# EPFL-VILAB/MultiMAE

Hardware: NVIDIA H100
Metric: MultiMAE-B pretrain samples/sec @ bs=128/GPU (higher is better)
Workload: dtype bf16

## Files before the change

multimae_b200/csrc/gemm_wgmma.cu:

```cuda
#include <algorithm>
#include <cstdlib>

#include "common.cuh"
#include "../../include/multimae_b200.h"

namespace mmae {

void count_launch();
bool gemm_profile_begin(cudaStream_t st, double flops, int M, int N, int K, int flags);
void gemm_profile_end(cudaStream_t st);

namespace {

constexpr int BM = 128;
constexpr int BK = 64;
constexpr int WG_K = 16;
constexpr int GEMM_THREADS = 384;

struct GemmParams {
  int M, N, K;
  int num_kb;
  int kb_per_split;
  int tiles_n;
  int tiles_m;
  int splits;
  int tma_store;
  mmae_gemm_epilogue ep;
};

template <int BN>
struct GemmCfg {
  static constexpr int STAGES = BN == 256 ? 4 : (BN == 192 ? 4 : (BN == 128 ? 6 : 8));
  static constexpr int A_BYTES = BM * BK * 2;
  static constexpr int B_BYTES = BN * BK * 2;
  static constexpr int STAGE_BYTES = A_BYTES + B_BYTES;
  static constexpr int EPI_BOX_BYTES = 64 * 32 * 4;
  static constexpr int EPI_OFFSET = STAGES * STAGE_BYTES;
  static constexpr int BAR_OFFSET = EPI_OFFSET + 2 * 2 * EPI_BOX_BYTES;
  static constexpr int TOTAL = BAR_OFFSET + 256 + 1024;
  static_assert(TOTAL <= 232448, "GEMM exceeds the 227 KB shared-memory limit");
};

struct WorkItem {
  int m0, n0, split, kb_begin, nkb;
};

template <int BN, int CL>
__device__ __forceinline__ WorkItem decode_item(int item, const GemmParams& p, int rank) {
  WorkItem w;
  const int rest = item / p.tiles_n;
  w.n0 = (item - rest * p.tiles_n) * BN;
  w.split = rest / p.tiles_m;
  w.m0 = ((rest - w.split * p.tiles_m) * CL + rank) * BM;
  w.kb_begin = w.split * p.kb_per_split;
  w.nkb = min(p.kb_per_split, p.num_kb - w.kb_begin);
  return w;
}

__device__ __forceinline__ void red_add_v2(float* addr, float a, float b) {
  asm volatile("red.global.add.v2.f32 [%0], {%1, %2};" ::"l"(addr), "f"(a), "f"(b) : "memory");
}

__device__ __forceinline__ void epilogue_pair(float v0, float v1, int row, int n, const GemmParams& p, bool first_split,
                                              bool atomic_out) {
  const mmae_gemm_epilogue& ep = p.ep;
  v0 *= ep.alpha;
  v1 *= ep.alpha;
  if (ep.bias && first_split) {
    const float2 b = __ldg(reinterpret_cast<const float2*>(ep.bias + n));
    v0 += b.x;
    v1 += b.y;
  }
  if (ep.preact_bf16)
    *reinterpret_cast<uint32_t*>(reinterpret_cast<bf16*>(ep.preact_bf16) + int64_t(row) * ep.ld_preact + n) = pack_bf16x2(v0, v1);
  if (ep.act == 1) {
    v0 = gelu_erf(v0);
    v1 = gelu_erf(v1);
  }
  if (ep.dgelu_z) {
    const uint32_t z = __ldg(reinterpret_cast<const unsigned int*>(reinterpret_cast<const bf16*>(ep.dgelu_z) +
                                                                   int64_t(row) * ep.ld_dgelu_z + n));
    const float2 zf = unpack_bf16x2(z);
    v0 *= dgelu_erf(zf.x);
    v1 *= dgelu_erf(zf.y);
  }
  if (ep.residual && first_split) {
    const float2 r = __ldg(reinterpret_cast<const float2*>(ep.residual + int64_t(row) * ep.ld_residual + n));
    v0 += r.x;
    v1 += r.y;
  }
  if (ep.out_f32) {
    float* dst = ep.out_f32 + int64_t(row) * ep.ld_out_f32 + n;
    if (atomic_out) red_add_v2(dst, v0, v1);
    else *reinterpret_cast<float2*>(dst) = make_float2(v0, v1);
  }
  if (ep.out_bf16)
    *reinterpret_cast<uint32_t*>(reinterpret_cast<bf16*>(ep.out_bf16) + int64_t(row) * ep.ld_out_bf16 + n) = pack_bf16x2(v0, v1);
}

template <typename T>
__device__ __forceinline__ void stage_pair(uint8_t* box, int r, int c, float v0, float v1) {
  T* b = reinterpret_cast<T*>(box);
  if constexpr (sizeof(T) == 4) *reinterpret_cast<float2*>(b + r * 32 + c) = make_float2(v0, v1);
  else *reinterpret_cast<uint32_t*>(b + r * 32 + c) = pack_bf16x2(v0, v1);
}

template <int BN, int CL, bool A_MN, bool B_MN>
__global__ void __launch_bounds__(GEMM_THREADS, 1)
    gemm_bf16_kernel(const __grid_constant__ CUtensorMap tmA, const __grid_constant__ CUtensorMap tmB,
                     const __grid_constant__ CUtensorMap tmC, const GemmParams p) {
  pdl_launch_dependents();
  using C = GemmCfg<BN>;
  constexpr int STAGES = C::STAGES;
  constexpr int BH = BN / CL;
  static_assert(!B_MN || BH % 64 == 0, "MN-major B is loaded in 64-column chunks");

  extern __shared__ uint8_t smem_raw[];
  const uint32_t raw_addr = smem_u32(smem_raw);
  uint8_t* smem = smem_raw + ((1024u - (raw_addr & 1023u)) & 1023u);
  uint64_t* full_bar = reinterpret_cast<uint64_t*>(smem + C::BAR_OFFSET);
  uint64_t* empty_bar = full_bar + STAGES;

  const int wg = threadIdx.x >> 7;
  const int rank = CL > 1 ? int(cluster_ctarank()) : 0;
  const int num_items = p.tiles_n * p.tiles_m * p.splits;
  const int first_item = blockIdx.x / CL;
  const int item_stride = gridDim.x / CL;

  if (threadIdx.x == 0) {
    tma_prefetch_desc(&tmA);
    tma_prefetch_desc(&tmB);
    if (p.tma_store) tma_prefetch_desc(&tmC);
#pragma unroll
    for (int s = 0; s < STAGES; ++s) {
      mbar_init(&full_bar[s], 1);
      mbar_init(&empty_bar[s], 2 * CL);
    }
    fence_barrier_init();
  }
  __syncthreads();
  if constexpr (CL > 1) cluster_sync_all();
  pdl_wait();

  if (wg == 0) {
    setmaxnreg_dec<40>();
    if (threadIdx.x == 0) {
      uint32_t it = 0;
      for (int item = first_item; item < num_items; item += item_stride) {
        const WorkItem w = decode_item<BN, CL>(item, p, rank);
        for (int kb = 0; kb < w.nkb; ++kb, ++it) {
          const int s = it % STAGES;
          const uint32_t ph = (it / STAGES) & 1;
          mbar_wait(&empty_bar[s], ph ^ 1u);
          mbar_expect_tx(&full_bar[s], C::STAGE_BYTES);
          uint8_t* sA = smem + s * C::STAGE_BYTES;
          uint8_t* sB = sA + C::A_BYTES;
          const int k0 = (w.kb_begin + kb) * BK;
          if constexpr (!A_MN) {
            tma_load_2d(sA, &tmA, &full_bar[s], k0, w.m0);
          } else {
#pragma unroll
            for (int c = 0; c < BM / 64; ++c) tma_load_2d(sA + c * (64 * BK * 2), &tmA, &full_bar[s], w.m0 + c * 64, k0);
          }
          if constexpr (CL == 1) {
            if constexpr (!B_MN) {
              tma_load_2d(sB, &tmB, &full_bar[s], k0, w.n0);
            } else {
#pragma unroll
              for (int c = 0; c < BN / 64; ++c) tma_load_2d(sB + c * (64 * BK * 2), &tmB, &full_bar[s], w.n0 + c * 64, k0);
            }
          } else {
            if constexpr (!B_MN) {
              tma_load_2d_multicast(sB + rank * BH * 128, &tmB, &full_bar[s], k0, w.n0 + rank * BH, 0x3);
            } else {
#pragma unroll
              for (int c = 0; c < BH / 64; ++c)
                tma_load_2d_multicast(sB + (rank * (BH / 64) + c) * (64 * BK * 2), &tmB, &full_bar[s],
                                      w.n0 + rank * BH + c * 64, k0, 0x3);
            }
          }
        }
      }
    }
  } else {
    setmaxnreg_inc<232>();
    const int cw = wg - 1;
    const int t = threadIdx.x & 127;
    const int rl = (t >> 5) * 16 + ((t & 31) >> 2);
    uint8_t* epi = smem + C::EPI_OFFSET + cw * (2 * C::EPI_BOX_BYTES);
    const bool atomic_out = p.ep.accumulate != 0 || p.splits > 1;
    uint32_t it = 0;
    uint32_t boxes = 0;
    auto release = [&](int s) {
      if (t == 0) {
        if constexpr (CL == 1) mbar_arrive(&empty_bar[s]);
        else
          for (int r = 0; r < CL; ++r) mbar_arrive_cluster(mapa_u32(smem_u32(&empty_bar[s]), uint32_t(r)));
      }
    };
    float acc[BN / 2];

    for (int item = first_item; item < num_items; item += item_stride) {
      const WorkItem w = decode_item<BN, CL>(item, p, rank);
      for (int kb = 0; kb < w.nkb; ++kb, ++it) {
        const int s = it % STAGES;
        const uint32_t ph = (it / STAGES) & 1;
        mbar_wait(&full_bar[s], ph);
        const uint32_t a_addr = smem_u32(smem + s * C::STAGE_BYTES) + cw * (64 * BK * 2);
        const uint32_t b_addr = smem_u32(smem + s * C::STAGE_BYTES) + C::A_BYTES;
#pragma unroll
        for (int i = 0; i < BN / 2; ++i) reg_fence(acc[i]);
        wgmma_fence();
#pragma unroll
        for (int j = 0; j < BK / WG_K; ++j) {
          const uint32_t sd = (kb | j) != 0 ? 1u : 0u;
          const uint64_t da = A_MN ? gmma_desc_sw128(a_addr + j * (WG_K * 128), 64 * BK * 2, 1024)
                                   : gmma_desc_sw128(a_addr + j * (WG_K * 2), 16, 1024);
          const uint64_t db = B_MN ? gmma_desc_sw128(b_addr + j * (WG_K * 128), 64 * BK * 2, 1024)
                                   : gmma_desc_sw128(b_addr + j * (WG_K * 2), 16, 1024);
          if constexpr (BN == 256) wgmma_m64n256k16<A_MN ? 1 : 0, B_MN ? 1 : 0>(acc, da, db, sd);
          else if constexpr (BN == 192) wgmma_m64n192k16<A_MN ? 1 : 0, B_MN ? 1 : 0>(acc, da, db, sd);
          else if constexpr (BN == 128) wgmma_m64n128k16<A_MN ? 1 : 0, B_MN ? 1 : 0>(acc, da, db, sd);
          else wgmma_m64n64k16<A_MN ? 1 : 0, B_MN ? 1 : 0>(acc, da, db, sd);
        }
        wgmma_commit();
#pragma unroll
        for (int i = 0; i < BN / 2; ++i) reg_fence(acc[i]);
        wgmma_wait<1>();
        if (kb > 0) release((it - 1) % STAGES);
      }
      wgmma_wait<0>();
#pragma unroll
      for (int i = 0; i < BN / 2; ++i) reg_fence(acc[i]);
      release((it - 1) % STAGES);

      const int row_a = w.m0 + cw * 64 + rl;
      const int row_b = row_a + 8;
      const bool first_split = w.split == 0;
      if (p.tma_store) {
        const float* bias = first_split ? p.ep.bias : nullptr;
        const bool bf16_out = p.tma_store == 1;
#pragma unroll
        for (int b = 0; b < BN / 32; ++b) {
          if (w.n0 + b * 32 >= p.N) break;
          uint8_t* box = bf16_out ? epi + (boxes & 3) * (C::EPI_BOX_BYTES / 2) : epi + (boxes & 1) * C::EPI_BOX_BYTES;
          if (t == 0) {
            if (bf16_out) bulk_wait_read<3>();
            else bulk_wait_read<1>();
          }
          asm volatile("bar.sync %0, 128;" ::"r"(2 + cw) : "memory");
#pragma unroll
          for (int jj = 0; jj < 4; ++jj) {
            const int j = 4 * b + jj;
            const int c = jj * 8 + 2 * (t & 3);
            float v[4] = {acc[4 * j] * p.ep.alpha, acc[4 * j + 1] * p.ep.alpha, acc[4 * j + 2] * p.ep.alpha,
                          acc[4 * j + 3] * p.ep.alpha};
            if (bias && w.n0 + b * 32 + c < p.N) {
              const float2 bb = __ldg(reinterpret_cast<const float2*>(bias + w.n0 + b * 32 + c));
              v[0] += bb.x; v[1] += bb.y; v[2] += bb.x; v[3] += bb.y;
            }
            if (p.ep.act == 1) {
#pragma unroll
              for (int i = 0; i < 4; ++i) v[i] = gelu_erf(v[i]);
            }
            if (bf16_out) {
              stage_pair<bf16>(box, rl, c, v[0], v[1]);
              stage_pair<bf16>(box, rl + 8, c, v[2], v[3]);
            } else {
              stage_pair<float>(box, rl, c, v[0], v[1]);
              stage_pair<float>(box, rl + 8, c, v[2], v[3]);
            }
          }
          fence_proxy_async_smem();
          asm volatile("bar.sync %0, 128;" ::"r"(2 + cw) : "memory");
          if (t == 0) {
            if (p.tma_store == 3) tma_reduce_add_2d(&tmC, box, w.n0 + b * 32, w.m0 + cw * 64);
            else tma_store_2d(&tmC, box, w.n0 + b * 32, w.m0 + cw * 64);
            bulk_commit_group();
          }
          ++boxes;
        }
      } else {
#pragma unroll
        for (int j = 0; j < BN / 8; ++j) {
          if (w.n0 + j * 8 >= p.N) break;
          const int n = w.n0 + j * 8 + 2 * (t & 3);
          if (row_a < p.M) epilogue_pair(acc[4 * j], acc[4 * j + 1], row_a, n, p, first_split, atomic_out);
          if (row_b < p.M) epilogue_pair(acc[4 * j + 2], acc[4 * j + 3], row_b, n, p, first_split, atomic_out);
        }
      }
    }
    if (t == 0 && p.tma_store) bulk_wait_all();
  }
  if constexpr (CL > 1) cluster_sync_all();
}

template <int BN, int CL, bool A_MN, bool B_MN>
int launch_gemm(const CUtensorMap& tmA, const CUtensorMap& tmB, const CUtensorMap& tmC, const GemmParams& p,
                cudaStream_t stream) {
  using C = GemmCfg<BN>;
  auto kern = gemm_bf16_kernel<BN, CL, A_MN, B_MN>;
  cudaLaunchConfig_t cfg;
  memset(&cfg, 0, sizeof(cfg));
  cfg.blockDim = dim3(GEMM_THREADS);
  cfg.dynamicSmemBytes = C::TOTAL;
  cfg.stream = stream;
  cudaLaunchAttribute attr[2];
  attr[0].id = cudaLaunchAttributeClusterDimension;
  attr[0].val.clusterDim.x = CL;
  attr[0].val.clusterDim.y = 1;
  attr[0].val.clusterDim.z = 1;
  attr[1].id = cudaLaunchAttributeProgrammaticStreamSerialization;
  attr[1].val.programmaticStreamSerializationAllowed = 1;
  cfg.attrs = attr;
  cfg.numAttrs = 1;
  static int resident = 0;
  if (resident == 0) {
    MMAE_CUDA_OK(cudaFuncSetAttribute(kern, cudaFuncAttributeMaxDynamicSharedMemorySize, C::TOTAL));
    if constexpr (CL > 1) {
      cfg.gridDim = dim3(CL);
      MMAE_CUDA_OK(cudaOccupancyMaxActiveClusters(&resident, kern, &cfg));
    } else {
      int dev = 0, sms = 0;
      MMAE_CUDA_OK(cudaGetDevice(&dev));
      MMAE_CUDA_OK(cudaDeviceGetAttribute(&sms, cudaDevAttrMultiProcessorCount, dev));
      resident = sms;
    }
    MMAE_CHECK(resident > 0, MMAE_ERR_CUDA, "mmae_gemm_bf16: the GEMM kernel does not fit on an SM");
  }
  const int items = p.tiles_n * p.tiles_m * p.splits;
  const int slots = std::min(resident, std::max(1, sm_count() / CL));
  cfg.gridDim = dim3(std::min(items, slots) * CL);
  const bool prof = gemm_profile_begin(stream, 2.0 * p.M * p.N * p.K, p.M, p.N, p.K,
                                       (A_MN ? 1 : 0) | (B_MN ? 2 : 0) | (p.splits << 8));
  if constexpr (CL == 1) {
    cfg.attrs = attr + 1;
    cfg.numAttrs = pdl_enabled() ? 1 : 0;
  } else {
    cfg.numAttrs = pdl_enabled() ? 2 : 1;
  }
  MMAE_CUDA_OK(cudaLaunchKernelEx(&cfg, kern, tmA, tmB, tmC, p));
  if (prof) gemm_profile_end(stream);
  count_launch();
  MMAE_LAUNCH_OK();
  return MMAE_OK;
}

}
}

using namespace mmae;

static int g_gemm_variant = []() {
  const char* e = getenv("MMAE_GEMM_VARIANT");
  const int v = e ? atoi(e) : -1;
  return v >= -1 && v <= 6 ? v : -1;
}();
static int g_gemm_tma_store = []() {
  const char* e = getenv("MMAE_GEMM_TMA_STORE");
  return e ? (atoi(e) != 0) : 1;
}();

extern "C" int mmae_gemm_set_variant(int variant) {
  MMAE_CHECK(variant >= -1 && variant <= 6, MMAE_ERR_ARG, "mmae_gemm_set_variant: %d (-1 .. 6)", variant);
  g_gemm_variant = variant;
  return MMAE_OK;
}

extern "C" int mmae_gemm_set_tma_store(int enable) {
  g_gemm_tma_store = enable != 0;
  return MMAE_OK;
}

static int variant_bn(int v) { return v == 0 ? 64 : (v == 1 || v == 6) ? 128 : (v == 3 || v == 5) ? 192 : 256; }

constexpr int KB_PER_ITEM_FIXED = 4;
constexpr int MIN_KB_PER_SPLIT = 16;

extern "C" int mmae_gemm_bf16(const void* A, int64_t lda, int a_mn_major, const void* B, int64_t ldb,
                              int b_mn_major, int M, int N, int K, int split_k, const mmae_gemm_epilogue* ep,
                              void* stream) {
  MMAE_CHECK(A && B && ep, MMAE_ERR_ARG, "mmae_gemm_bf16: null operand");
  MMAE_CHECK(M > 0 && N > 0 && K > 0, MMAE_ERR_ARG, "mmae_gemm_bf16: bad shape M=%d N=%d K=%d", M, N, K);
  MMAE_CHECK(N % 8 == 0, MMAE_ERR_ARG, "mmae_gemm_bf16: N=%d must be a multiple of 8", N);
  MMAE_CHECK(lda % 8 == 0 && ldb % 8 == 0, MMAE_ERR_ARG, "mmae_gemm_bf16: lda/ldb must be multiples of 8");
  MMAE_CHECK((reinterpret_cast<uintptr_t>(A) & 15) == 0 && (reinterpret_cast<uintptr_t>(B) & 15) == 0,
             MMAE_ERR_ARG, "mmae_gemm_bf16: operands must be 16-byte aligned");
  MMAE_CHECK(ep->out_f32 || ep->out_bf16, MMAE_ERR_ARG, "mmae_gemm_bf16: no output");
  const int num_kb = ceil_div(K, BK);
  const int sms = sm_count();
  const int tm = ceil_div(M, BM);
  if (split_k <= 0 && !(ep->out_f32 && !ep->out_bf16 && !ep->preact_bf16 && !ep->dgelu_z && ep->act == 0)) split_k = 1;

  int variant = g_gemm_variant;
  {
    const int cand_var[2] = {1, 2};
    const int nvar = variant >= 0 ? 1 : 2;
    long best_cost = -1;
    int best_split = 1, best_var = variant >= 0 ? variant : 1;
    for (int i = 0; i < nvar; ++i) {
      const int v = variant >= 0 ? variant : cand_var[i];
      const int bn = variant_bn(v), cl = v >= 4 ? 2 : 1;
      if (variant < 0 && bn > 128 && N < bn) continue;
      const long tiles = long(ceil_div(tm, cl)) * ceil_div(N, bn);
      const int slots = std::max(1, sms / cl);
      const int s_lo = split_k > 0 ? split_k : 1;
      const int s_hi = split_k > 0 ? split_k : std::max(1, num_kb / MIN_KB_PER_SPLIT);
      for (int s = s_lo; s <= s_hi; ++s) {
        const int kbps = ceil_div(num_kb, std::min(s, num_kb));
        const long rounds = (tiles * ceil_div(num_kb, kbps) + slots - 1) / slots;
        const long cost = rounds * (bn + 40) * cl * (kbps + KB_PER_ITEM_FIXED);
        if (best_cost < 0 || cost < best_cost) {
          best_cost = cost;
          best_split = s;
          best_var = v;
        }
      }
    }
    split_k = best_split;
    variant = best_var;
  }
  if (split_k > num_kb) split_k = num_kb;
  const int kb_per_split = ceil_div(num_kb, split_k);
  split_k = ceil_div(num_kb, kb_per_split);
  if (split_k > 1 || ep->accumulate) {
    MMAE_CHECK(ep->out_f32 && !ep->out_bf16 && !ep->preact_bf16 && !ep->dgelu_z && ep->act == 0, MMAE_ERR_ARG,
               "mmae_gemm_bf16: split-K / accumulate supports only a linear fp32 epilogue");
  }
#define MMAE_LD_OK(ptr, ld) (!(ptr) || ((ld) % 8 == 0 && (reinterpret_cast<uintptr_t>(ptr) & 15) == 0))
  MMAE_CHECK(MMAE_LD_OK(ep->residual, ep->ld_residual) && MMAE_LD_OK(ep->dgelu_z, ep->ld_dgelu_z) &&
                 MMAE_LD_OK(ep->preact_bf16, ep->ld_preact) && MMAE_LD_OK(ep->out_f32, ep->ld_out_f32) &&
                 MMAE_LD_OK(ep->out_bf16, ep->ld_out_bf16) &&
                 (!ep->bias || (reinterpret_cast<uintptr_t>(ep->bias) & 15) == 0),
             MMAE_ERR_ARG, "mmae_gemm_bf16: epilogue tensors need 16-byte alignment and ld %% 8 == 0");
#undef MMAE_LD_OK

  if (variant == 5 && b_mn_major) variant = 4;
  const int BNsel = variant_bn(variant);
  const int CLsel = variant >= 4 ? 2 : 1;

  CUtensorMap tmA, tmB;
  int rc;
  if (!a_mn_major) {
    rc = make_tmap_2d_bf16(&tmA, A, (uint64_t)M, (uint64_t)K, (uint64_t)lda, BK, BM);
  } else {
    MMAE_CHECK(M % 8 == 0, MMAE_ERR_ARG, "mmae_gemm_bf16: MN-major A needs M %% 8 == 0");
    rc = make_tmap_2d_bf16(&tmA, A, (uint64_t)K, (uint64_t)M, (uint64_t)lda, 64, BK);
  }
  if (rc) return rc;
  if (!b_mn_major) {
    rc = make_tmap_2d_bf16(&tmB, B, (uint64_t)N, (uint64_t)K, (uint64_t)ldb, BK, BNsel / CLsel);
  } else {
    rc = make_tmap_2d_bf16(&tmB, B, (uint64_t)K, (uint64_t)N, (uint64_t)ldb, 64, BK);
  }
  if (rc) return rc;

  GemmParams p;
  p.M = M; p.N = N; p.K = K;
  p.num_kb = num_kb;
  p.kb_per_split = kb_per_split;
  p.tiles_n = ceil_div(N, BNsel);
  p.tiles_m = ceil_div(tm, CLsel);
  p.splits = split_k;
  p.ep = *ep;
  p.tma_store = 0;
  CUtensorMap tmC = tmA;
  if (g_gemm_tma_store && !ep->preact_bf16 && !ep->dgelu_z && !ep->residual) {
    if (ep->out_bf16 && !ep->out_f32 && split_k == 1 && !ep->accumulate) {
      p.tma_store = 1;
      rc = make_tmap_2d_store(&tmC, ep->out_bf16, 2, (uint64_t)M, (uint64_t)N, (uint64_t)ep->ld_out_bf16);
      if (rc) return rc;
    } else if (ep->out_f32 && !ep->out_bf16 && ep->act == 0) {
      p.tma_store = (split_k > 1 || ep->accumulate) ? 3 : 2;
      rc = make_tmap_2d_store(&tmC, ep->out_f32, 4, (uint64_t)M, (uint64_t)N, (uint64_t)ep->ld_out_f32);
      if (rc) return rc;
    }
  }
  cudaStream_t st = reinterpret_cast<cudaStream_t>(stream);
#define MMAE_DISPATCH(BN_, CL_)                                                                      \
  do {                                                                                               \
    if (!a_mn_major && !b_mn_major) return launch_gemm<BN_, CL_, false, false>(tmA, tmB, tmC, p, st); \
    if (!a_mn_major && b_mn_major) return launch_gemm<BN_, CL_, false, true>(tmA, tmB, tmC, p, st);   \
    if (a_mn_major && !b_mn_major) return launch_gemm<BN_, CL_, true, false>(tmA, tmB, tmC, p, st);   \
    return launch_gemm<BN_, CL_, true, true>(tmA, tmB, tmC, p, st);                                  \
  } while (0)
  if (variant == 4) MMAE_DISPATCH(256, 2);
  if (variant == 6) MMAE_DISPATCH(128, 2);
  if (variant == 5) {
    if (!a_mn_major) return launch_gemm<192, 2, false, false>(tmA, tmB, tmC, p, st);
    return launch_gemm<192, 2, true, false>(tmA, tmB, tmC, p, st);
  }
  if (variant == 0) MMAE_DISPATCH(64, 1);
  if (variant == 3) MMAE_DISPATCH(192, 1);
  if (variant == 2) MMAE_DISPATCH(256, 1);
  MMAE_DISPATCH(128, 1);
#undef MMAE_DISPATCH
}
```

multimae_b200/csrc/runtime.cu:

```cuda
#include <atomic>
#include <cstdarg>
#include <cstdio>
#include <cstring>
#include <vector>

#include "common.cuh"
#include "../../include/multimae_b200.h"

namespace mmae {

static thread_local char g_err[512] = "";
static std::atomic<int64_t> g_launches{0};

void set_last_error(const char* fmt, ...) {
  va_list ap;
  va_start(ap, fmt);
  vsnprintf(g_err, sizeof(g_err), fmt, ap);
  va_end(ap);
}

void count_launch() { g_launches.fetch_add(1, std::memory_order_relaxed); }

struct GemmProfile {
  bool on = false;
  std::vector<cudaEvent_t> begin, end;
  std::vector<double> flops;
  std::vector<long long> shape;
  size_t used = 0;
};
static GemmProfile g_prof;
static const size_t kProfCap = 8192;

bool gemm_profile_begin(cudaStream_t st, double flops, int M, int N, int K, int flags) {
  if (!g_prof.on || g_prof.used >= kProfCap) return false;
  if (g_prof.begin.size() <= g_prof.used) {
    cudaEvent_t a, b;
    if (cudaEventCreate(&a) != cudaSuccess || cudaEventCreate(&b) != cudaSuccess) return false;
    g_prof.begin.push_back(a);
    g_prof.end.push_back(b);
    g_prof.flops.push_back(0.0);
    for (int i = 0; i < 4; ++i) g_prof.shape.push_back(0);
  }
  g_prof.flops[g_prof.used] = flops;
  g_prof.shape[4 * g_prof.used + 0] = M;
  g_prof.shape[4 * g_prof.used + 1] = N;
  g_prof.shape[4 * g_prof.used + 2] = K;
  g_prof.shape[4 * g_prof.used + 3] = flags;
  cudaEventRecord(g_prof.begin[g_prof.used], st);
  return true;
}
void gemm_profile_end(cudaStream_t st) {
  cudaEventRecord(g_prof.end[g_prof.used], st);
  g_prof.used++;
}

static int g_sm_budget = []() {
  const char* e = getenv("MMAE_SM_BUDGET");
  return e ? atoi(e) : 0;
}();
int sm_count() {
  static int cached = 0;
  if (cached == 0) {
    int dev = 0;
    cudaGetDevice(&dev);
    cudaDeviceGetAttribute(&cached, cudaDevAttrMultiProcessorCount, dev);
    if (cached <= 0) cached = 132;
  }
  return g_sm_budget > 0 && g_sm_budget < cached ? g_sm_budget : cached;
}

typedef CUresult (*encode_tiled_fn)(CUtensorMap*, CUtensorMapDataType, cuuint32_t, void*, const cuuint64_t*,
                                    const cuuint64_t*, const cuuint32_t*, const cuuint32_t*,
                                    CUtensorMapInterleave, CUtensorMapSwizzle, CUtensorMapL2promotion,
                                    CUtensorMapFloatOOBfill);

static encode_tiled_fn get_encode_fn() {
  static encode_tiled_fn fn = nullptr;
  if (!fn) {
    void* p = nullptr;
    cudaDriverEntryPointQueryResult q;
    cudaError_t e = cudaGetDriverEntryPoint("cuTensorMapEncodeTiled", &p, cudaEnableDefault, &q);
    if (e != cudaSuccess || q != cudaDriverEntryPointSuccess || !p) {
      set_last_error("cuTensorMapEncodeTiled entry point unavailable (%s)", cudaGetErrorString(e));
      return nullptr;
    }
    fn = reinterpret_cast<encode_tiled_fn>(p);
  }
  return fn;
}

int make_tmap_2d_bf16(CUtensorMap* out, const void* base, uint64_t rows, uint64_t cols, uint64_t ld,
                      uint32_t box_cols, uint32_t box_rows) {
  encode_tiled_fn fn = get_encode_fn();
  if (!fn) return MMAE_ERR_CUDA;
  cuuint64_t dims[2] = {cols, rows};
  cuuint64_t strides[1] = {ld * 2};
  cuuint32_t box[2] = {box_cols, box_rows};
  cuuint32_t estr[2] = {1, 1};
  CUresult r = fn(out, CU_TENSOR_MAP_DATA_TYPE_BFLOAT16, 2, const_cast<void*>(base), dims, strides, box, estr,
                  CU_TENSOR_MAP_INTERLEAVE_NONE, CU_TENSOR_MAP_SWIZZLE_128B, CU_TENSOR_MAP_L2_PROMOTION_L2_256B,
                  CU_TENSOR_MAP_FLOAT_OOB_FILL_NONE);
  if (r != CUDA_SUCCESS) {
    set_last_error("cuTensorMapEncodeTiled(2d) failed: %d (rows=%llu cols=%llu ld=%llu box=%ux%u base=%p)", (int)r,
                   (unsigned long long)rows, (unsigned long long)cols, (unsigned long long)ld, box_cols, box_rows,
                   base);
    return MMAE_ERR_CUDA;
  }
  return MMAE_OK;
}

int make_tmap_2d_store(CUtensorMap* out, const void* base, int elem_bytes, uint64_t rows, uint64_t cols, uint64_t ld) {
  encode_tiled_fn fn = get_encode_fn();
  if (!fn) return MMAE_ERR_CUDA;
  cuuint64_t dims[2] = {cols, rows};
  cuuint64_t strides[1] = {ld * (uint64_t)elem_bytes};
  cuuint32_t box[2] = {32, 64};
  cuuint32_t estr[2] = {1, 1};
  CUresult r = fn(out, elem_bytes == 2 ? CU_TENSOR_MAP_DATA_TYPE_BFLOAT16 : CU_TENSOR_MAP_DATA_TYPE_FLOAT32, 2,
                  const_cast<void*>(base), dims, strides, box, estr,
                  CU_TENSOR_MAP_INTERLEAVE_NONE, CU_TENSOR_MAP_SWIZZLE_NONE, CU_TENSOR_MAP_L2_PROMOTION_NONE,
                  CU_TENSOR_MAP_FLOAT_OOB_FILL_NONE);
  if (r != CUDA_SUCCESS) {
    set_last_error("cuTensorMapEncodeTiled(store) failed: %d (rows=%llu cols=%llu ld=%llu base=%p)", (int)r,
                   (unsigned long long)rows, (unsigned long long)cols, (unsigned long long)ld, base);
    return MMAE_ERR_CUDA;
  }
  return MMAE_OK;
}

int make_tmap_3d_bf16(CUtensorMap* out, const void* base, uint64_t d0, uint64_t d1, uint64_t d2, uint64_t s1,
                      uint64_t s2, uint32_t b0, uint32_t b1, uint32_t b2) {
  encode_tiled_fn fn = get_encode_fn();
  if (!fn) return MMAE_ERR_CUDA;
  cuuint64_t dims[3] = {d0, d1, d2};
  cuuint64_t strides[2] = {s1 * 2, s2 * 2};
  cuuint32_t box[3] = {b0, b1, b2};
  cuuint32_t estr[3] = {1, 1, 1};
  CUresult r = fn(out, CU_TENSOR_MAP_DATA_TYPE_BFLOAT16, 3, const_cast<void*>(base), dims, strides, box, estr,
                  CU_TENSOR_MAP_INTERLEAVE_NONE, CU_TENSOR_MAP_SWIZZLE_128B, CU_TENSOR_MAP_L2_PROMOTION_L2_256B,
                  CU_TENSOR_MAP_FLOAT_OOB_FILL_NONE);
  if (r != CUDA_SUCCESS) {
    set_last_error("cuTensorMapEncodeTiled(3d) failed: %d", (int)r);
    return MMAE_ERR_CUDA;
  }
  return MMAE_OK;
}

int make_tmap_3d_bf16_store(CUtensorMap* out, const void* base, uint64_t d0, uint64_t d1, uint64_t d2, uint64_t s1,
                            uint64_t s2, uint32_t b0, uint32_t b1, uint32_t b2) {
  encode_tiled_fn fn = get_encode_fn();
  if (!fn) return MMAE_ERR_CUDA;
  cuuint64_t dims[3] = {d0, d1, d2};
  cuuint64_t strides[2] = {s1 * 2, s2 * 2};
  cuuint32_t box[3] = {b0, b1, b2};
  cuuint32_t estr[3] = {1, 1, 1};
  const CUtensorMapSwizzle sw = b0 * 2 == 128 ? CU_TENSOR_MAP_SWIZZLE_128B : (b0 * 2 == 64 ? CU_TENSOR_MAP_SWIZZLE_64B : CU_TENSOR_MAP_SWIZZLE_NONE);
  CUresult r = fn(out, CU_TENSOR_MAP_DATA_TYPE_BFLOAT16, 3, const_cast<void*>(base), dims, strides, box, estr,
                  CU_TENSOR_MAP_INTERLEAVE_NONE, sw, CU_TENSOR_MAP_L2_PROMOTION_NONE, CU_TENSOR_MAP_FLOAT_OOB_FILL_NONE);
  if (r != CUDA_SUCCESS) {
    set_last_error("cuTensorMapEncodeTiled(3d store) failed: %d", (int)r);
    return MMAE_ERR_CUDA;
  }
  return MMAE_OK;
}

}

namespace mmae {
namespace {
struct MirrorEntry {
  const float* f32;
  bf16* b16;
  int64_t n;
};
constexpr int MAX_MIRRORS = 8;
MirrorEntry g_mirror[MAX_MIRRORS];
int g_num_mirrors = 0;
}

const bf16* mirror_lookup(const float* w) {
  for (int i = 0; i < g_num_mirrors; ++i) {
    const MirrorEntry& e = g_mirror[i];
    if (w >= e.f32 && w < e.f32 + e.n) {
      const int64_t off = w - e.f32;
      if (off % 8 != 0) return nullptr;
      return e.b16 + off;
    }
  }
  return nullptr;
}
}

extern "C" int mmae_weight_mirror_register(const float* params_f32, void* mirror_bf16, int64_t n) {
  using namespace mmae;
  MMAE_CHECK(params_f32 != nullptr, MMAE_ERR_ARG, "mmae_weight_mirror_register: null parameter buffer");
  int at = -1;
  for (int i = 0; i < g_num_mirrors; ++i)
    if (g_mirror[i].f32 == params_f32) at = i;
  if (mirror_bf16 == nullptr || n <= 0) {
    if (at >= 0) g_mirror[at] = g_mirror[--g_num_mirrors];
    return MMAE_OK;
  }
  MMAE_CHECK((reinterpret_cast<uintptr_t>(params_f32) & 31) == 0 && (reinterpret_cast<uintptr_t>(mirror_bf16) & 15) == 0,
             MMAE_ERR_ARG, "mmae_weight_mirror_register: buffers must be 32-byte (fp32) / 16-byte (bf16) aligned");
  if (at < 0) {
    MMAE_CHECK(g_num_mirrors < MAX_MIRRORS, MMAE_ERR_UNSUPPORTED, "mmae_weight_mirror_register: too many mirrors");
    at = g_num_mirrors++;
  }
  g_mirror[at] = {params_f32, reinterpret_cast<bf16*>(mirror_bf16), n};
  return MMAE_OK;
}

namespace mmae {
static int g_pdl = []() {
  const char* e = getenv("MMAE_PDL");
  return e ? atoi(e) : 0;
}();
bool pdl_enabled() { return g_pdl != 0; }
}
extern "C" int mmae_set_sm_budget(int sms) {
  mmae::g_sm_budget = sms;
  return MMAE_OK;
}
extern "C" int mmae_set_pdl(int enable) {
  mmae::g_pdl = enable != 0;
  return MMAE_OK;
}

extern "C" int mmae_abi_version(void) { return MMAE_ABI_VERSION; }
extern "C" const char* mmae_last_error(void) { return mmae::g_err; }
extern "C" int64_t mmae_launch_count(void) { return mmae::g_launches.load(std::memory_order_relaxed); }

extern "C" int mmae_profile_gemm(int enable) {
  mmae::g_prof.on = enable != 0;
  if (enable) mmae::g_prof.used = 0;
  return MMAE_OK;
}
extern "C" int mmae_profile_gemm_read(double* flops, double* ms, int64_t* launches) {
  double f = 0.0, t = 0.0;
  for (size_t i = 0; i < mmae::g_prof.used; ++i) {
    if (cudaEventSynchronize(mmae::g_prof.end[i]) != cudaSuccess) return MMAE_ERR_CUDA;
    float e = 0.f;
    if (cudaEventElapsedTime(&e, mmae::g_prof.begin[i], mmae::g_prof.end[i]) != cudaSuccess) return MMAE_ERR_CUDA;
    t += e;
    f += mmae::g_prof.flops[i];
  }
  if (flops) *flops = f;
  if (ms) *ms = t;
  if (launches) *launches = (int64_t)mmae::g_prof.used;
  return MMAE_OK;
}

extern "C" int64_t mmae_profile_gemm_dump(char* buf, int64_t cap) {
  int64_t off = 0;
  for (size_t i = 0; i < mmae::g_prof.used; ++i) {
    if (cudaEventSynchronize(mmae::g_prof.end[i]) != cudaSuccess) return -1;
    float e = 0.f;
    cudaEventElapsedTime(&e, mmae::g_prof.begin[i], mmae::g_prof.end[i]);
    const int n = snprintf(buf + off, (size_t)(cap - off), "%lld %lld %lld %lld %.6f\n", mmae::g_prof.shape[4 * i],
                           mmae::g_prof.shape[4 * i + 1], mmae::g_prof.shape[4 * i + 2], mmae::g_prof.shape[4 * i + 3], e);
    if (n <= 0 || off + n >= cap) break;
    off += n;
  }
  return off;
}
```

Baseline: 3886.

## Swizzle TMA-store epilogue boxes and lend a pipeline stage for BN=256 staging

```diff
diff --git a/multimae_b200/csrc/gemm_wgmma.cu b/multimae_b200/csrc/gemm_wgmma.cu
--- a/multimae_b200/csrc/gemm_wgmma.cu
+++ b/multimae_b200/csrc/gemm_wgmma.cu
@@ -31,12 +31,13 @@
 template <int BN>
 struct GemmCfg {
   static constexpr int STAGES = BN == 256 ? 4 : (BN == 192 ? 4 : (BN == 128 ? 6 : 8));
+  static constexpr int EPI_BOXES = 2;
   static constexpr int A_BYTES = BM * BK * 2;
   static constexpr int B_BYTES = BN * BK * 2;
   static constexpr int STAGE_BYTES = A_BYTES + B_BYTES;
-  static constexpr int EPI_BOX_BYTES = 64 * 32 * 4;
+  static constexpr int EPI_BOX_BYTES = 64 * 128;
   static constexpr int EPI_OFFSET = STAGES * STAGE_BYTES;
-  static constexpr int BAR_OFFSET = EPI_OFFSET + 2 * 2 * EPI_BOX_BYTES;
+  static constexpr int BAR_OFFSET = EPI_OFFSET + 2 * EPI_BOXES * EPI_BOX_BYTES;
   static constexpr int TOTAL = BAR_OFFSET + 256 + 1024;
   static_assert(TOTAL <= 232448, "GEMM exceeds the 227 KB shared-memory limit");
 };
@@ -100,9 +101,60 @@
 
 template <typename T>
 __device__ __forceinline__ void stage_pair(uint8_t* box, int r, int c, float v0, float v1) {
-  T* b = reinterpret_cast<T*>(box);
-  if constexpr (sizeof(T) == 4) *reinterpret_cast<float2*>(b + r * 32 + c) = make_float2(v0, v1);
-  else *reinterpret_cast<uint32_t*>(b + r * 32 + c) = pack_bf16x2(v0, v1);
+  const int byte = c * int(sizeof(T));
+  uint8_t* dst = box + r * 128 + ((((byte >> 4) ^ r) & 7) << 4) + (byte & 15);
+  if constexpr (sizeof(T) == 4) *reinterpret_cast<float2*>(dst) = make_float2(v0, v1);
+  else *reinterpret_cast<uint32_t*>(dst) = pack_bf16x2(v0, v1);
+}
+
+template <typename T, int BN, int NBOX, int NLENT>
+__device__ __forceinline__ void tma_epilogue(const float (&acc)[BN / 2], const CUtensorMap* tmC, uint8_t* epi,
+                                             uint8_t* lent, const GemmParams& p, const float* bias, int m0, int n0,
+                                             int rl, int t, int bar_id, uint32_t& boxes) {
+  constexpr int BOX_COLS = 128 / int(sizeof(T));
+  constexpr int BOX_BYTES = 64 * 128;
+  static_assert(NBOX >= 2, "the staging area holds at least two boxes");
+  static_assert(NLENT == 0 || BN / BOX_COLS <= NLENT + NBOX, "an item's boxes fit in the lent and own staging boxes");
+  if constexpr (NLENT == 0) {
+    if (t == 0) bulk_wait_read<NBOX - 1>();
+  }
+  asm volatile("bar.sync %0, 128;" ::"r"(bar_id) : "memory");
+#pragma unroll
+  for (int b = 0; b < BN / BOX_COLS; ++b) {
+    const int c0 = n0 + b * BOX_COLS;
+    if (c0 >= p.N) break;
+    uint8_t* box = NLENT == 0 ? epi + (boxes % NBOX) * BOX_BYTES
+                              : (b < NLENT ? lent + b * BOX_BYTES : epi + (b - NLENT) * BOX_BYTES);
+#pragma unroll
+    for (int jj = 0; jj < BOX_COLS / 8; ++jj) {
+      const int j = b * (BOX_COLS / 8) + jj;
+      const int c = jj * 8 + 2 * (t & 3);
+      float v[4] = {acc[4 * j] * p.ep.alpha, acc[4 * j + 1] * p.ep.alpha, acc[4 * j + 2] * p.ep.alpha,
+                    acc[4 * j + 3] * p.ep.alpha};
+      if (bias && c0 + c < p.N) {
+        const float2 bb = __ldg(reinterpret_cast<const float2*>(bias + c0 + c));
+        v[0] += bb.x; v[1] += bb.y; v[2] += bb.x; v[3] += bb.y;
+      }
+      if (p.ep.act == 1) {
+#pragma unroll
+        for (int i = 0; i < 4; ++i) v[i] = gelu_erf(v[i]);
+      }
+      stage_pair<T>(box, rl, c, v[0], v[1]);
+      stage_pair<T>(box, rl + 8, c, v[2], v[3]);
+    }
+    fence_proxy_async_smem();
+    if (t == 0 && b + 1 < BN / BOX_COLS && c0 + BOX_COLS < p.N) {
+      if constexpr (NLENT == 0) bulk_wait_read<NBOX - 2>();
+      else if (b + 1 == NLENT) bulk_wait_read<NLENT - 1>();
+    }
+    asm volatile("bar.sync %0, 128;" ::"r"(bar_id) : "memory");
+    if (t == 0) {
+      if (p.tma_store == 3) tma_reduce_add_2d(tmC, box, c0, m0);
+      else tma_store_2d(tmC, box, c0, m0);
+      bulk_commit_group();
+    }
+    ++boxes;
+  }
 }
 
 template <int BN, int CL, bool A_MN, bool B_MN>
@@ -187,10 +239,14 @@
     const int cw = wg - 1;
     const int t = threadIdx.x & 127;
     const int rl = (t >> 5) * 16 + ((t & 31) >> 2);
-    uint8_t* epi = smem + C::EPI_OFFSET + cw * (2 * C::EPI_BOX_BYTES);
+    uint8_t* epi = smem + C::EPI_OFFSET + cw * (C::EPI_BOXES * C::EPI_BOX_BYTES);
     const bool atomic_out = p.ep.accumulate != 0 || p.splits > 1;
     uint32_t it = 0;
     uint32_t boxes = 0;
+    constexpr int NLENT = BN == 256 ? 2 : 0;
+    const bool lend = NLENT > 0 && p.tma_store == 1;
+    int lent_stage = -1;
+    int lent_after = 0;
     auto release = [&](int s) {
       if (t == 0) {
         if constexpr (CL == 1) mbar_arrive(&empty_bar[s]);
@@ -228,57 +284,39 @@
         for (int i = 0; i < BN / 2; ++i) reg_fence(acc[i]);
         wgmma_wait<1>();
         if (kb > 0) release((it - 1) % STAGES);
+        if (kb == 0 && lent_stage >= 0) {
+          if (t == 0) {
+            if (lent_after >= 2) bulk_wait_read<2>();
+            else if (lent_after == 1) bulk_wait_read<1>();
+            else bulk_wait_read<0>();
+          }
+          release(lent_stage);
+          lent_stage = -1;
+        }
       }
       wgmma_wait<0>();
 #pragma unroll
       for (int i = 0; i < BN / 2; ++i) reg_fence(acc[i]);
-      release((it - 1) % STAGES);
+      if (lend) {
+        lent_stage = (it - 1) % STAGES;
+        asm volatile("bar.sync 1, 256;" ::: "memory");
+      } else {
+        release((it - 1) % STAGES);
+      }
 
       const int row_a = w.m0 + cw * 64 + rl;
       const int row_b = row_a + 8;
       const bool first_split = w.split == 0;
       if (p.tma_store) {
         const float* bias = first_split ? p.ep.bias : nullptr;
-        const bool bf16_out = p.tma_store == 1;
-#pragma unroll
-        for (int b = 0; b < BN / 32; ++b) {
-          if (w.n0 + b * 32 >= p.N) break;
-          uint8_t* box = bf16_out ? epi + (boxes & 3) * (C::EPI_BOX_BYTES / 2) : epi + (boxes & 1) * C::EPI_BOX_BYTES;
-          if (t == 0) {
-            if (bf16_out) bulk_wait_read<3>();
-            else bulk_wait_read<1>();
-          }
-          asm volatile("bar.sync %0, 128;" ::"r"(2 + cw) : "memory");
-#pragma unroll
-          for (int jj = 0; jj < 4; ++jj) {
-            const int j = 4 * b + jj;
-            const int c = jj * 8 + 2 * (t & 3);
-            float v[4] = {acc[4 * j] * p.ep.alpha, acc[4 * j + 1] * p.ep.alpha, acc[4 * j + 2] * p.ep.alpha,
-                          acc[4 * j + 3] * p.ep.alpha};
-            if (bias && w.n0 + b * 32 + c < p.N) {
-              const float2 bb = __ldg(reinterpret_cast<const float2*>(bias + w.n0 + b * 32 + c));
-              v[0] += bb.x; v[1] += bb.y; v[2] += bb.x; v[3] += bb.y;
-            }
-            if (p.ep.act == 1) {
-#pragma unroll
-              for (int i = 0; i < 4; ++i) v[i] = gelu_erf(v[i]);
-            }
-            if (bf16_out) {
-              stage_pair<bf16>(box, rl, c, v[0], v[1]);
-              stage_pair<bf16>(box, rl + 8, c, v[2], v[3]);
-            } else {
-              stage_pair<float>(box, rl, c, v[0], v[1]);
-              stage_pair<float>(box, rl + 8, c, v[2], v[3]);
-            }
-          }
-          fence_proxy_async_smem();
-          asm volatile("bar.sync %0, 128;" ::"r"(2 + cw) : "memory");
-          if (t == 0) {
-            if (p.tma_store == 3) tma_reduce_add_2d(&tmC, box, w.n0 + b * 32, w.m0 + cw * 64);
-            else tma_store_2d(&tmC, box, w.n0 + b * 32, w.m0 + cw * 64);
-            bulk_commit_group();
-          }
-          ++boxes;
+        if (p.tma_store == 1) {
+          uint8_t* lent = lend ? smem + lent_stage * C::STAGE_BYTES + cw * (C::STAGE_BYTES / 2) : nullptr;
+          tma_epilogue<bf16, BN, C::EPI_BOXES, NLENT>(acc, &tmC, epi, lent, p, bias, w.m0 + cw * 64, w.n0, rl, t, 2 + cw,
+                                                      boxes);
+          lent_after = max(0, min(BN / 64, (p.N - w.n0 + 63) / 64) - NLENT);
+        } else {
+          tma_epilogue<float, BN, C::EPI_BOXES, 0>(acc, &tmC, epi, nullptr, p, bias, w.m0 + cw * 64, w.n0, rl, t, 2 + cw,
+                                                   boxes);
         }
       } else {
 #pragma unroll
diff --git a/multimae_b200/csrc/runtime.cu b/multimae_b200/csrc/runtime.cu
--- a/multimae_b200/csrc/runtime.cu
+++ b/multimae_b200/csrc/runtime.cu
@@ -114,11 +114,11 @@
   if (!fn) return MMAE_ERR_CUDA;
   cuuint64_t dims[2] = {cols, rows};
   cuuint64_t strides[1] = {ld * (uint64_t)elem_bytes};
-  cuuint32_t box[2] = {32, 64};
+  cuuint32_t box[2] = {128u / (uint32_t)elem_bytes, 64};
   cuuint32_t estr[2] = {1, 1};
   CUresult r = fn(out, elem_bytes == 2 ? CU_TENSOR_MAP_DATA_TYPE_BFLOAT16 : CU_TENSOR_MAP_DATA_TYPE_FLOAT32, 2,
                   const_cast<void*>(base), dims, strides, box, estr,
-                  CU_TENSOR_MAP_INTERLEAVE_NONE, CU_TENSOR_MAP_SWIZZLE_NONE, CU_TENSOR_MAP_L2_PROMOTION_NONE,
+                  CU_TENSOR_MAP_INTERLEAVE_NONE, CU_TENSOR_MAP_SWIZZLE_128B, CU_TENSOR_MAP_L2_PROMOTION_NONE,
                   CU_TENSOR_MAP_FLOAT_OOB_FILL_NONE);
   if (r != CUDA_SUCCESS) {
     set_last_error("cuTensorMapEncodeTiled(store) failed: %d (rows=%llu cols=%llu ld=%llu base=%p)", (int)r,
```

New measurement: 3933, median of 6. 1.2% higher.
